# hassony2/handobjectconsist

Measured on AMD Instinct MI355X. Metric: trainmeshwarp iters/sec (render+warp, B=64, 256x256), higher is better.
Workload: dtype f32; 1 GPU; trainmeshwarp.py consist step, per-GPU B=64, 256x256, hand 778v/1552f + object 1002v/2000f (7104 faces after fill-back), ResNet-18 fp32 (MIOpen convolutions, channels-last, + fused HIP BatchNorm/ReLU/residual/max-pool kernels), Adam; global_batch=64, image_size=256, parallelism=dp1

## Files before the change

handobjectconsist_amd/csrc/frozen_bn.hip:

```cpp
#include "mr_common.hpp"

namespace mr {

__device__ __forceinline__ float relu_nan(float z) { return z > 0.0f ? z : (z != z ? z : 0.0f); }


struct BnParams {
    const void* x;
    const void* residual;
    const float* weight;
    const float* bias;
    const float* mean;
    const float* var;
    float eps;
    int relu;
    int N, C, HW, split;
    void* y;
    const void* grad_y;
    const void* grad_y2;
    void* grad_x;
    void* grad_residual;
    float* partial;
};

typedef unsigned short bf16_t;
__device__ __forceinline__ float to_f32(float v) { return v; }
__device__ __forceinline__ float to_f32(bf16_t v) { return __uint_as_float((unsigned)v << 16); }
template <typename T> __device__ __forceinline__ T from_f32(float v);
template <> __device__ __forceinline__ float from_f32<float>(float v) { return v; }
template <> __device__ __forceinline__ bf16_t from_f32<bf16_t>(float v) {
    unsigned u = __float_as_uint(v);
    if ((u & 0x7fffffffu) > 0x7f800000u) return (bf16_t)0x7fc0;
    u += 0x7fffu + ((u >> 16) & 1u);
    return (bf16_t)(u >> 16);
}
template <typename T> struct Vec4;
template <> struct Vec4<float> { typedef float4 type; };
template <> struct Vec4<bf16_t> { typedef ushort4 type; };

template <typename T>
__device__ __forceinline__ void load4(const void* base, int64_t o, float* v) {
    const typename Vec4<T>::type t = *reinterpret_cast<const typename Vec4<T>::type*>(static_cast<const T*>(base) + o);
    v[0] = to_f32(t.x); v[1] = to_f32(t.y); v[2] = to_f32(t.z); v[3] = to_f32(t.w);
}
template <typename T>
__device__ __forceinline__ void store4(void* base, int64_t o, const float* v) {
    typename Vec4<T>::type t;
    t.x = from_f32<T>(v[0]); t.y = from_f32<T>(v[1]); t.z = from_f32<T>(v[2]); t.w = from_f32<T>(v[3]);
    *reinterpret_cast<typename Vec4<T>::type*>(static_cast<T*>(base) + o) = t;
}

__device__ __forceinline__ void channel_consts(const BnParams& p, int c, float& mean, float& a, float& b, float& invstd) {
    mean = p.mean[c];
    invstd = 1.0f / sqrtf(p.var[c] + p.eps);
    a = p.weight[c] * invstd;
    b = p.bias[c];
}

template <typename T, bool VEC, bool BACKWARD>
__global__ __launch_bounds__(256) void bn_act_kernel(BnParams p) {
    const int c = blockIdx.x / p.split, k = blockIdx.x % p.split;
    const int n0 = (int)((int64_t)k * p.N / p.split), n1 = (int)((int64_t)(k + 1) * p.N / p.split);
    float mean, a, b, invstd;
    channel_consts(p, c, mean, a, b, invstd);
    constexpr int W = VEC ? 4 : 1;
    const int per_plane = p.HW / W;
    const unsigned total = (unsigned)(n1 - n0) * (unsigned)per_plane;
    const bool relu = p.relu != 0;
    float sum_g = 0.0f, sum_gx = 0.0f;
    for (unsigned e = threadIdx.x; e < total; e += 256) {
        const unsigned q = e / (unsigned)per_plane;
        const int n = n0 + (int)q, j = (int)(e - q * (unsigned)per_plane);
        const int64_t o = ((int64_t)n * p.C + c) * p.HW + (int64_t)j * W;
        float xv[W], rv[W], gv[W];
        if (VEC) {
            load4<T>(p.x, o, xv);
            if (p.residual) load4<T>(p.residual, o, rv);
            if (BACKWARD) {
                load4<T>(p.grad_y, o, gv);
                if (p.grad_y2) {
                    float g2[4];
                    load4<T>(p.grad_y2, o, g2);
#pragma unroll
                    for (int i = 0; i < 4; i++) gv[i] += g2[i];
                }
            }
        } else {
            xv[0] = to_f32(static_cast<const T*>(p.x)[o]);
            if (p.residual) rv[0] = to_f32(static_cast<const T*>(p.residual)[o]);
            if (BACKWARD) {
                gv[0] = to_f32(static_cast<const T*>(p.grad_y)[o]);
                if (p.grad_y2) gv[0] += to_f32(static_cast<const T*>(p.grad_y2)[o]);
            }
        }
        float out[W], gres[W];
#pragma unroll
        for (int i = 0; i < W; i++) {
            const float d = xv[i] - mean;
            float z = d * a + b;
            if (p.residual) z = z + rv[i];
            if (!BACKWARD) {
                out[i] = relu ? relu_nan(z) : z;
            } else {
                const float g = (relu && !(z > 0.0f)) ? 0.0f : gv[i];
                gres[i] = g;
                out[i] = g * a;
                sum_g += g;
                sum_gx += g * d;
            }
        }
        void* dst = BACKWARD ? p.grad_x : p.y;
        if (VEC) {
            store4<T>(dst, o, out);
            if (BACKWARD && p.grad_residual) store4<T>(p.grad_residual, o, gres);
        } else {
            static_cast<T*>(dst)[o] = from_f32<T>(out[0]);
            if (BACKWARD && p.grad_residual) static_cast<T*>(p.grad_residual)[o] = from_f32<T>(gres[0]);
        }
    }
    if (BACKWARD && p.partial) {
        __shared__ float red[2][4];
#pragma unroll
        for (int off = 32; off >= 1; off >>= 1) {
            sum_g += __shfl_down(sum_g, off);
            sum_gx += __shfl_down(sum_gx, off);
        }
        const int wave = threadIdx.x >> 6;
        if ((threadIdx.x & 63) == 0) { red[0][wave] = sum_g; red[1][wave] = sum_gx; }
        __syncthreads();
        if (threadIdx.x == 0) {
            p.partial[(int64_t)c * p.split + k] = (red[0][0] + red[0][1]) + (red[0][2] + red[0][3]);
            p.partial[(int64_t)(p.C + c) * p.split + k] = (red[1][0] + red[1][1]) + (red[1][2] + red[1][3]);
        }
    }
}

__global__ __launch_bounds__(256) void bn_finish_kernel(const float* __restrict__ partial, const float* __restrict__ var,
                                                        float eps, float* grad_weight, float* grad_bias, int C, int split) {
    __shared__ float red[2][4];
    const int c = blockIdx.x;
    float s0 = 0.0f, s1 = 0.0f;
    for (int k = threadIdx.x; k < split; k += 256) {
        s0 += partial[(int64_t)c * split + k];
        s1 += partial[(int64_t)(C + c) * split + k];
    }
#pragma unroll
    for (int off = 32; off >= 1; off >>= 1) {
        s0 += __shfl_down(s0, off);
        s1 += __shfl_down(s1, off);
    }
    if ((threadIdx.x & 63) == 0) { red[0][threadIdx.x >> 6] = s0; red[1][threadIdx.x >> 6] = s1; }
    __syncthreads();
    if (threadIdx.x == 0) {
        if (grad_bias) grad_bias[c] = (red[0][0] + red[0][1]) + (red[0][2] + red[0][3]);
        if (grad_weight) grad_weight[c] = ((red[1][0] + red[1][1]) + (red[1][2] + red[1][3])) * (1.0f / sqrtf(var[c] + eps));
    }
}

constexpr int BN_NHWC_BLOCKS = 2048;

template <typename T, bool BACKWARD>
__global__ __launch_bounds__(256) void bn_act_nhwc_kernel(BnParams p) {
    __shared__ float red[256][9];
    const int groups = p.C >> 2;
    const int cg = threadIdx.x % groups, prow = threadIdx.x / groups, rows = 256 / groups;
    const int c0 = 4 * cg;
    float mean[4], a[4], b[4];
#pragma unroll
    for (int i = 0; i < 4; i++) {
        float invstd;
        channel_consts(p, c0 + i, mean[i], a[i], b[i], invstd);
    }
    const int64_t pixels = (int64_t)p.N * p.HW;
    const bool relu = p.relu != 0;
    float sg[4] = {0.0f, 0.0f, 0.0f, 0.0f}, sgx[4] = {0.0f, 0.0f, 0.0f, 0.0f};
    for (int64_t px = (int64_t)blockIdx.x * rows + prow; px < pixels; px += (int64_t)gridDim.x * rows) {
        const int64_t o = px * p.C + c0;
        float xv[4], rv[4], gv[4], out[4], gres[4];
        load4<T>(p.x, o, xv);
        if (p.residual) load4<T>(p.residual, o, rv);
        if (BACKWARD) {
            load4<T>(p.grad_y, o, gv);
            if (p.grad_y2) {
                float g2[4];
                load4<T>(p.grad_y2, o, g2);
#pragma unroll
                for (int i = 0; i < 4; i++) gv[i] += g2[i];
            }
        }
#pragma unroll
        for (int i = 0; i < 4; i++) {
            const float d = xv[i] - mean[i];
            float z = d * a[i] + b[i];
            if (p.residual) z = z + rv[i];
            if (!BACKWARD) {
                out[i] = relu ? relu_nan(z) : z;
            } else {
                const float g = (relu && !(z > 0.0f)) ? 0.0f : gv[i];
                gres[i] = g;
                out[i] = g * a[i];
                sg[i] += g;
                sgx[i] += g * d;
            }
        }
        store4<T>(BACKWARD ? p.grad_x : p.y, o, out);
        if (BACKWARD && p.grad_residual) store4<T>(p.grad_residual, o, gres);
    }
    if (BACKWARD && p.partial) {
#pragma unroll
        for (int i = 0; i < 4; i++) { red[threadIdx.x][i] = sg[i]; red[threadIdx.x][4 + i] = sgx[i]; }
        __syncthreads();
        if (threadIdx.x < groups) {
            float t[8] = {0, 0, 0, 0, 0, 0, 0, 0};
            for (int r = 0; r < rows; r++)
#pragma unroll
                for (int i = 0; i < 8; i++) t[i] += red[r * groups + threadIdx.x][i];
#pragma unroll
            for (int i = 0; i < 4; i++) {
                p.partial[(int64_t)(c0 + i) * gridDim.x + blockIdx.x] = t[i];
                p.partial[(int64_t)(p.C + c0 + i) * gridDim.x + blockIdx.x] = t[4 + i];
            }
        }
    }
}

static inline bool bn_nhwc_ok(int C) { return C >= 4 && C <= 1024 && (1024 % C) == 0; }

static inline int bn_nhwc_blocks(int64_t pixels, int C) {
    const int rows = 256 / (C / 4);
    const int64_t need = (pixels + rows - 1) / rows;
    return (int)(need < BN_NHWC_BLOCKS ? (need < 1 ? 1 : need) : BN_NHWC_BLOCKS);
}

static inline int bn_split(int N, int C) {
    int s = (4096 + C - 1) / C;
    if (s < 1) s = 1;
    if (s > N) s = N;
    return s;
}

static inline bool bn_aligned(const void* p, int bytes) { return (reinterpret_cast<uintptr_t>(p) & (uintptr_t)(bytes - 1)) == 0; }

template <bool BACKWARD>
static void bn_launch(const BnParams& p, int act_dtype, bool vec, hipStream_t s) {
    const dim3 grid((unsigned)(p.C * p.split));
    if (act_dtype == 0) {
        if (vec) hipLaunchKernelGGL((bn_act_kernel<float, true, BACKWARD>), grid, dim3(256), 0, s, p);
        else hipLaunchKernelGGL((bn_act_kernel<float, false, BACKWARD>), grid, dim3(256), 0, s, p);
    } else {
        if (vec) hipLaunchKernelGGL((bn_act_kernel<bf16_t, true, BACKWARD>), grid, dim3(256), 0, s, p);
        else hipLaunchKernelGGL((bn_act_kernel<bf16_t, false, BACKWARD>), grid, dim3(256), 0, s, p);
    }
}

}

extern "C" int mr_bn_act_forward(const void* x, const void* residual, const float* weight, const float* bias,
                                 const float* running_mean, const float* running_var, float eps, int relu, int act_dtype,
                                 int channels_last, void* y, int batch_size, int channels, int plane,
                                 mr_stream_t stream) {
    using namespace mr;
    if (batch_size < 0 || channels < 0 || plane < 0 || (act_dtype != 0 && act_dtype != 1)) return MR_ERR_BADARG;
    if (channels_last && channels > 0 && !bn_nhwc_ok(channels)) return MR_ERR_BADARG;
    if (batch_size == 0 || channels == 0 || plane == 0) return MR_OK;
    if (!x || !weight || !bias || !running_mean || !running_var || !y) return MR_ERR_BADARG;
    BnParams p{};
    p.x = x; p.residual = residual; p.weight = weight; p.bias = bias; p.mean = running_mean; p.var = running_var;
    p.eps = eps; p.relu = relu; p.N = batch_size; p.C = channels; p.HW = plane; p.split = bn_split(batch_size, channels);
    p.y = y;
    if ((int64_t)channels * p.split > 0x7fffffff || ((int64_t)batch_size / p.split + 1) * plane > 0x7fffffff) return MR_ERR_BADARG;
    const int vb = act_dtype == 0 ? 16 : 8;
    if (channels_last) {
        if (!bn_aligned(x, vb) || !bn_aligned(y, vb) || !bn_aligned(residual, vb)) return MR_ERR_BADARG;
        const dim3 grid((unsigned)bn_nhwc_blocks((int64_t)batch_size * plane, channels));
        if (act_dtype == 0) hipLaunchKernelGGL((bn_act_nhwc_kernel<float, false>), grid, dim3(256), 0, (hipStream_t)stream, p);
        else hipLaunchKernelGGL((bn_act_nhwc_kernel<bf16_t, false>), grid, dim3(256), 0, (hipStream_t)stream, p);
        MR_CHECK_LAUNCH();
        return MR_OK;
    }
    const bool vec = plane % 4 == 0 && bn_aligned(x, vb) && bn_aligned(y, vb) && bn_aligned(residual, vb);
    bn_launch<false>(p, act_dtype, vec, (hipStream_t)stream);
    MR_CHECK_LAUNCH();
    return MR_OK;
}

extern "C" int64_t mr_bn_act_backward_workspace_bytes(int batch_size, int channels) {
    if (batch_size < 0 || channels < 0) return -1;
    const int64_t split = mr::bn_split(batch_size > 0 ? batch_size : 1, channels > 0 ? channels : 1);
    return (int64_t)2 * channels * (split > mr::BN_NHWC_BLOCKS ? split : mr::BN_NHWC_BLOCKS) * 4 + 16;
}

extern "C" int mr_bn_act_backward(const void* grad_y, const void* grad_y2, const void* x, const void* residual,
                                  const float* weight,
                                  const float* bias, const float* running_mean, const float* running_var, float eps,
                                  int relu, int act_dtype, int channels_last, void* grad_x, void* grad_residual,
                                  float* grad_weight, float* grad_bias, void* workspace, int64_t workspace_bytes,
                                  int batch_size, int channels, int plane, mr_stream_t stream) {
    using namespace mr;
    if (batch_size < 0 || channels < 0 || plane < 0 || (act_dtype != 0 && act_dtype != 1)) return MR_ERR_BADARG;
    if (channels_last && channels > 0 && !bn_nhwc_ok(channels)) return MR_ERR_BADARG;
    if (channels == 0) return MR_OK;
    if (!weight || !bias || !running_mean || !running_var) return MR_ERR_BADARG;
    const bool want_params = grad_weight || grad_bias;
    if (batch_size == 0 || plane == 0) {
        hipError_t e = hipSuccess;
        if (grad_weight) e = hipMemsetAsync(grad_weight, 0, (size_t)channels * 4, (hipStream_t)stream);
        if (e == hipSuccess && grad_bias) e = hipMemsetAsync(grad_bias, 0, (size_t)channels * 4, (hipStream_t)stream);
        return e == hipSuccess ? MR_OK : (int)e;
    }
    if (!grad_y || !x || !grad_x) return MR_ERR_BADARG;
    if (grad_residual && !residual) return MR_ERR_BADARG;
    if (want_params && (!workspace || workspace_bytes < mr_bn_act_backward_workspace_bytes(batch_size, channels)))
        return MR_ERR_BADARG;
    BnParams p{};
    p.x = x; p.residual = residual; p.weight = weight; p.bias = bias; p.mean = running_mean; p.var = running_var;
    p.eps = eps; p.relu = relu; p.N = batch_size; p.C = channels; p.HW = plane; p.split = bn_split(batch_size, channels);
    p.grad_y = grad_y; p.grad_y2 = grad_y2; p.grad_x = grad_x; p.grad_residual = grad_residual;
    p.partial = want_params ? static_cast<float*>(workspace) : nullptr;
    if ((int64_t)channels * p.split > 0x7fffffff || ((int64_t)batch_size / p.split + 1) * plane > 0x7fffffff) return MR_ERR_BADARG;
    const int vb = act_dtype == 0 ? 16 : 8;
    int slots = p.split;
    if (channels_last) {
        if (!bn_aligned(x, vb) || !bn_aligned(grad_y, vb) || !bn_aligned(grad_y2, vb) || !bn_aligned(grad_x, vb) ||
            !bn_aligned(residual, vb) ||
            !bn_aligned(grad_residual, vb))
            return MR_ERR_BADARG;
        slots = bn_nhwc_blocks((int64_t)batch_size * plane, channels);
        const dim3 grid((unsigned)slots);
        if (act_dtype == 0) hipLaunchKernelGGL((bn_act_nhwc_kernel<float, true>), grid, dim3(256), 0, (hipStream_t)stream, p);
        else hipLaunchKernelGGL((bn_act_nhwc_kernel<bf16_t, true>), grid, dim3(256), 0, (hipStream_t)stream, p);
    } else {
        const bool vec = plane % 4 == 0 && bn_aligned(x, vb) && bn_aligned(grad_y, vb) && bn_aligned(grad_y2, vb) &&
                         bn_aligned(grad_x, vb) &&
                         bn_aligned(residual, vb) && bn_aligned(grad_residual, vb);
        bn_launch<true>(p, act_dtype, vec, (hipStream_t)stream);
    }
    MR_CHECK_LAUNCH();
    if (want_params) {
        hipLaunchKernelGGL(bn_finish_kernel, dim3((unsigned)channels), dim3(256), 0, (hipStream_t)stream, p.partial,
                           running_var, eps, grad_weight, grad_bias, channels, slots);
        MR_CHECK_LAUNCH();
    }
    return MR_OK;
}
```

handobjectconsist_amd/csrc/stem_pool.hip:

```cpp
#include "mr_common.hpp"

namespace mr {

__device__ __forceinline__ float sp_relu_nan(float z) { return z > 0.0f ? z : (z != z ? z : 0.0f); }


struct StemParams {
    const void* x;
    const float* weight;
    const float* bias;
    const float* mean;
    const float* var;
    float eps;
    int N, C, H, W, OH, OW;
    int tiles_x, tiles_y;
    void* y;
    const void* grad_y;
    const void* grad_y2;
    void* grad_x;
    float* partial;
    unsigned char* argmax;
};

constexpr int SP_TX = 32, SP_TY = 16;
constexpr int SP_IH = 2 * SP_TY + 3, SP_IW = 2 * SP_TX + 8, SP_C0 = 4;
constexpr int SP_LDW = SP_IW + 1;

typedef unsigned short bf16_t;
__device__ __forceinline__ float sp_f32(float v) { return v; }
__device__ __forceinline__ float sp_f32(bf16_t v) { return __uint_as_float((unsigned)v << 16); }
template <typename T> __device__ __forceinline__ T sp_from(float v);
template <> __device__ __forceinline__ float sp_from<float>(float v) { return v; }
template <> __device__ __forceinline__ bf16_t sp_from<bf16_t>(float v) {
    unsigned u = __float_as_uint(v);
    if ((u & 0x7fffffffu) > 0x7f800000u) return (bf16_t)0x7fc0;
    u += 0x7fffu + ((u >> 16) & 1u);
    return (bf16_t)(u >> 16);
}
template <typename T> struct SpVec4;
template <> struct SpVec4<float> { typedef float4 type; };
template <> struct SpVec4<bf16_t> { typedef ushort4 type; };

__device__ __forceinline__ void stem_consts(const StemParams& p, int c, float& mean, float& a, float& b) {
    mean = p.mean[c];
    a = p.weight[c] * (1.0f / sqrtf(p.var[c] + p.eps));
    b = p.bias[c];
}

template <typename T, bool KEEP_D>
__device__ __forceinline__ void load_tile(const StemParams& p, const T* xp, int oy0, int ox0, float mean, float a,
                                          float b, float (*zt)[SP_LDW], float (*dt)[SP_LDW]) {
    const int iy0 = 2 * oy0 - 1, ix0 = 2 * ox0 - SP_C0;
    const float ninf = -__builtin_inff();
    if ((p.W & 3) == 0 && (reinterpret_cast<uintptr_t>(xp) & (4 * sizeof(T) - 1)) == 0) {
        for (int e = threadIdx.x; e < SP_IH * (SP_IW / 4); e += 256) {
            const int r = e / (SP_IW / 4), q = e - r * (SP_IW / 4);
            const int iy = iy0 + r, ix = ix0 + 4 * q;
            float v[4] = {0.0f, 0.0f, 0.0f, 0.0f};
            const bool in = iy >= 0 && iy < p.H && ix >= 0 && ix < p.W;
            if (in) {
                const typename SpVec4<T>::type t = *reinterpret_cast<const typename SpVec4<T>::type*>(xp + (int64_t)iy * p.W + ix);
                v[0] = sp_f32(t.x); v[1] = sp_f32(t.y); v[2] = sp_f32(t.z); v[3] = sp_f32(t.w);
            }
#pragma unroll
            for (int i = 0; i < 4; i++) {
                const float d = v[i] - mean;
                zt[r][4 * q + i] = in ? d * a + b : ninf;
                if (KEEP_D) dt[r][4 * q + i] = in ? d : 0.0f;
            }
        }
        return;
    }
    for (int e = threadIdx.x; e < SP_IH * SP_IW; e += 256) {
        const int r = e / SP_IW, c = e - r * SP_IW;
        const int iy = iy0 + r, ix = ix0 + c;
        float z = ninf, d = 0.0f;
        if (iy >= 0 && iy < p.H && ix >= 0 && ix < p.W) {
            d = sp_f32(xp[(int64_t)iy * p.W + ix]) - mean;
            z = d * a + b;
        }
        zt[r][c] = z;
        if (KEEP_D) dt[r][c] = d;
    }
}

template <typename T>
__global__ __launch_bounds__(256) void stem_pool_forward_kernel(StemParams p) {
    __shared__ float zt[SP_IH][SP_LDW];
    const int tiles = p.tiles_x * p.tiles_y;
    const int plane = blockIdx.x / tiles, t = blockIdx.x % tiles;
    const int c = plane % p.C;
    const int oy0 = (t / p.tiles_x) * SP_TY, ox0 = (t % p.tiles_x) * SP_TX;
    float mean, a, b;
    stem_consts(p, c, mean, a, b);
    load_tile<T, false>(p, static_cast<const T*>(p.x) + (int64_t)plane * p.H * p.W, oy0, ox0, mean, a, b, zt, nullptr);
    __syncthreads();
    for (int e = threadIdx.x; e < SP_TY * SP_TX; e += 256) {
        const int wy = e / SP_TX, wx = e % SP_TX;
        const int oy = oy0 + wy, ox = ox0 + wx;
        if (oy >= p.OH || ox >= p.OW) continue;
        float m = 0.0f;
#pragma unroll
        for (int kh = 0; kh < 3; kh++)
#pragma unroll
            for (int kw = 0; kw < 3; kw++) {
                const float z = zt[2 * wy + kh][2 * wx + kw + SP_C0 - 1];
                m = (z > m || z != z) ? z : m;
            }
        static_cast<T*>(p.y)[((int64_t)plane * p.OH + oy) * p.OW + ox] = sp_from<T>(m);
    }
}

template <typename T>
__global__ __launch_bounds__(256) void stem_pool_backward_kernel(StemParams p) {
    __shared__ float zt[SP_IH][SP_LDW];
    __shared__ float dt[SP_IH][SP_LDW];
    __shared__ float gw[SP_TY + 1][SP_TX + 1];
    __shared__ unsigned char am[SP_TY + 1][SP_TX + 1];
    __shared__ float red[2][4];
    const int tiles = p.tiles_x * p.tiles_y;
    const int plane = blockIdx.x / tiles, t = blockIdx.x % tiles;
    const int c = plane % p.C;
    const int oy0 = (t / p.tiles_x) * SP_TY, ox0 = (t % p.tiles_x) * SP_TX;
    float mean, a, b;
    stem_consts(p, c, mean, a, b);
    const T* xp = static_cast<const T*>(p.x) + (int64_t)plane * p.H * p.W;
    load_tile<T, true>(p, xp, oy0, ox0, mean, a, b, zt, dt);
    __syncthreads();
    for (int e = threadIdx.x; e < (SP_TY + 1) * (SP_TX + 1); e += 256) {
        const int wy = e / (SP_TX + 1), wx = e - wy * (SP_TX + 1);
        const int oy = oy0 + wy, ox = ox0 + wx;
        float g = 0.0f;
        int best = 0;
        if (oy < p.OH && ox < p.OW) {
            g = sp_f32(static_cast<const T*>(p.grad_y)[((int64_t)plane * p.OH + oy) * p.OW + ox]);
            if (p.grad_y2) g += sp_f32(static_cast<const T*>(p.grad_y2)[((int64_t)plane * p.OH + oy) * p.OW + ox]);
            float mv = -__builtin_inff();
#pragma unroll
            for (int k = 0; k < 9; k++) {
                const float z = zt[2 * wy + k / 3][2 * wx + k % 3 + SP_C0 - 1];
                const float v = sp_relu_nan(z);
                if (z != -__builtin_inff() && (v > mv || v != v)) { mv = v; best = k; }
            }
        }
        gw[wy][wx] = g;
        am[wy][wx] = (unsigned char)best;
    }
    __syncthreads();
    float sum_g = 0.0f, sum_gx = 0.0f;
    T* gx = static_cast<T*>(p.grad_x) + (int64_t)plane * p.H * p.W;
    const bool vec = (p.W & 3) == 0 && (reinterpret_cast<uintptr_t>(gx) & (4 * sizeof(T) - 1)) == 0;
    for (int e = threadIdx.x; e < 2 * SP_TY * (2 * SP_TX / 4); e += 256) {
        const int ry = e / (2 * SP_TX / 4), rx0 = 4 * (e - ry * (2 * SP_TX / 4));
        const int iy = 2 * oy0 + ry, ix0 = 2 * ox0 + rx0;
        if (iy >= p.H || ix0 >= p.W) continue;
        const int ly = ry + 1;
        float out[4];
#pragma unroll
        for (int i = 0; i < 4; i++) {
            const int lx = rx0 + i + 1;
            float g = 0.0f;
#pragma unroll
            for (int dy = 0; dy < 2; dy++) {
                const int wy = (ly >> 1) - dy;
                const int kh = ly - 2 * wy;
                if (wy < 0 || kh > 2) continue;
#pragma unroll
                for (int dx = 0; dx < 2; dx++) {
                    const int wx = (lx >> 1) - dx;
                    const int kw = lx - 2 * wx;
                    if (wx < 0 || kw > 2) continue;
                    if (am[wy][wx] == kh * 3 + kw) g += gw[wy][wx];
                }
            }
            const float z = zt[ly][lx + SP_C0 - 1];
            const float gm = (z > 0.0f && ix0 + i < p.W) ? g : 0.0f;
            out[i] = gm * a;
            sum_g += gm;
            sum_gx += gm * dt[ly][lx + SP_C0 - 1];
        }
        T* dst = gx + (int64_t)iy * p.W + ix0;
        if (vec) {
            typename SpVec4<T>::type t;
            t.x = sp_from<T>(out[0]); t.y = sp_from<T>(out[1]); t.z = sp_from<T>(out[2]); t.w = sp_from<T>(out[3]);
            *reinterpret_cast<typename SpVec4<T>::type*>(dst) = t;
        } else {
#pragma unroll
            for (int i = 0; i < 4; i++)
                if (ix0 + i < p.W) dst[i] = sp_from<T>(out[i]);
        }
    }
    if (p.partial) {
#pragma unroll
        for (int off = 32; off >= 1; off >>= 1) {
            sum_g += __shfl_down(sum_g, off);
            sum_gx += __shfl_down(sum_gx, off);
        }
        const int wave = threadIdx.x >> 6;
        if ((threadIdx.x & 63) == 0) { red[0][wave] = sum_g; red[1][wave] = sum_gx; }
        __syncthreads();
        if (threadIdx.x == 0) {
            const int n = plane / p.C;
            const int64_t per_c = (int64_t)p.N * tiles;
            const int64_t slot = (int64_t)n * tiles + t;
            p.partial[(int64_t)c * per_c + slot] = (red[0][0] + red[0][1]) + (red[0][2] + red[0][3]);
            p.partial[((int64_t)p.C + c) * per_c + slot] = (red[1][0] + red[1][1]) + (red[1][2] + red[1][3]);
        }
    }
}

__global__ __launch_bounds__(256) void stem_finish_kernel(const float* __restrict__ partial, const float* __restrict__ var,
                                                          float eps, float* grad_weight, float* grad_bias, int C,
                                                          int64_t per_c) {
    __shared__ float red[2][4];
    const int c = blockIdx.x;
    float s0 = 0.0f, s1 = 0.0f;
    for (int64_t k = threadIdx.x; k < per_c; k += 256) {
        s0 += partial[(int64_t)c * per_c + k];
        s1 += partial[((int64_t)C + c) * per_c + k];
    }
#pragma unroll
    for (int off = 32; off >= 1; off >>= 1) {
        s0 += __shfl_down(s0, off);
        s1 += __shfl_down(s1, off);
    }
    if ((threadIdx.x & 63) == 0) { red[0][threadIdx.x >> 6] = s0; red[1][threadIdx.x >> 6] = s1; }
    __syncthreads();
    if (threadIdx.x == 0) {
        if (grad_bias) grad_bias[c] = (red[0][0] + red[0][1]) + (red[0][2] + red[0][3]);
        if (grad_weight) grad_weight[c] = ((red[1][0] + red[1][1]) + (red[1][2] + red[1][3])) * (1.0f / sqrtf(var[c] + eps));
    }
}

constexpr int SP_NHWC_BLOCKS = 4096;

template <typename T>
__device__ __forceinline__ void sp_load4(const T* base, int64_t o, float* v) {
    const typename SpVec4<T>::type t = *reinterpret_cast<const typename SpVec4<T>::type*>(base + o);
    v[0] = sp_f32(t.x); v[1] = sp_f32(t.y); v[2] = sp_f32(t.z); v[3] = sp_f32(t.w);
}
template <typename T>
__device__ __forceinline__ void sp_store4(T* base, int64_t o, const float* v) {
    typename SpVec4<T>::type t;
    t.x = sp_from<T>(v[0]); t.y = sp_from<T>(v[1]); t.z = sp_from<T>(v[2]); t.w = sp_from<T>(v[3]);
    *reinterpret_cast<typename SpVec4<T>::type*>(base + o) = t;
}

template <typename T>
__global__ __launch_bounds__(256) void stem_pool_nhwc_forward_kernel(StemParams p) {
    const int groups = p.C >> 2, cg = threadIdx.x % groups, prow = threadIdx.x / groups, rows = 256 / groups;
    const int c0 = 4 * cg;
    float mean[4], a[4], b[4];
#pragma unroll
    for (int i = 0; i < 4; i++) stem_consts(p, c0 + i, mean[i], a[i], b[i]);
    const T* x = static_cast<const T*>(p.x);
    const int64_t total = (int64_t)p.N * p.OH * p.OW;
    for (int64_t op = (int64_t)blockIdx.x * rows + prow; op < total; op += (int64_t)gridDim.x * rows) {
        const int ox = (int)(op % p.OW), oy = (int)((op / p.OW) % p.OH), n = (int)(op / ((int64_t)p.OW * p.OH));
        float best[4];
        unsigned bi[4] = {0, 0, 0, 0};
#pragma unroll
        for (int i = 0; i < 4; i++) best[i] = -__builtin_inff();
#pragma unroll
        for (int k = 0; k < 9; k++) {
            const int iy = 2 * oy - 1 + k / 3, ix = 2 * ox - 1 + k % 3;
            if (iy < 0 || iy >= p.H || ix < 0 || ix >= p.W) continue;
            float xv[4];
            sp_load4<T>(x, (((int64_t)n * p.H + iy) * p.W + ix) * p.C + c0, xv);
#pragma unroll
            for (int i = 0; i < 4; i++) {
                const float v = sp_relu_nan((xv[i] - mean[i]) * a[i] + b[i]);
                if (v > best[i] || v != v) { best[i] = v; bi[i] = (unsigned)k; }
            }
        }
        const int64_t o = op * p.C + c0;
        sp_store4<T>(static_cast<T*>(p.y), o, best);
        *reinterpret_cast<uchar4*>(p.argmax + o) = make_uchar4((unsigned char)bi[0], (unsigned char)bi[1],
                                                               (unsigned char)bi[2], (unsigned char)bi[3]);
    }
}

template <typename T>
__global__ __launch_bounds__(256) void stem_pool_nhwc_backward_kernel(StemParams p) {
    __shared__ float red[256][9];
    const int groups = p.C >> 2, cg = threadIdx.x % groups, prow = threadIdx.x / groups, rows = 256 / groups;
    const int c0 = 4 * cg;
    float mean[4], a[4], b[4];
#pragma unroll
    for (int i = 0; i < 4; i++) stem_consts(p, c0 + i, mean[i], a[i], b[i]);
    const T* x = static_cast<const T*>(p.x);
    const T* gy = static_cast<const T*>(p.grad_y);
    const T* gy2 = static_cast<const T*>(p.grad_y2);
    const int64_t total = (int64_t)p.N * p.H * p.W;
    float sg[4] = {0.0f, 0.0f, 0.0f, 0.0f}, sgx[4] = {0.0f, 0.0f, 0.0f, 0.0f};
    for (int64_t ip = (int64_t)blockIdx.x * rows + prow; ip < total; ip += (int64_t)gridDim.x * rows) {
        const int ix = (int)(ip % p.W), iy = (int)((ip / p.W) % p.H), n = (int)(ip / ((int64_t)p.W * p.H));
        float xv[4], g[4] = {0.0f, 0.0f, 0.0f, 0.0f}, out[4];
        sp_load4<T>(x, ip * p.C + c0, xv);
        const int ly = iy + 1, lx = ix + 1;
#pragma unroll
        for (int dy = 0; dy < 2; dy++) {
            const int wy = (ly >> 1) - dy, kh = ly - 2 * wy;
            if (wy < 0 || wy >= p.OH || kh > 2) continue;
#pragma unroll
            for (int dx = 0; dx < 2; dx++) {
                const int wx = (lx >> 1) - dx, kw = lx - 2 * wx;
                if (wx < 0 || wx >= p.OW || kw > 2) continue;
                const int64_t o = (((int64_t)n * p.OH + wy) * p.OW + wx) * p.C + c0;
                const uchar4 id = *reinterpret_cast<const uchar4*>(p.argmax + o);
                float gv[4];
                sp_load4<T>(gy, o, gv);
                if (gy2) {
                    float g2[4];
                    sp_load4<T>(gy2, o, g2);
#pragma unroll
                    for (int i = 0; i < 4; i++) gv[i] += g2[i];
                }
                const unsigned code = (unsigned)(kh * 3 + kw);
                g[0] += id.x == code ? gv[0] : 0.0f;
                g[1] += id.y == code ? gv[1] : 0.0f;
                g[2] += id.z == code ? gv[2] : 0.0f;
                g[3] += id.w == code ? gv[3] : 0.0f;
            }
        }
#pragma unroll
        for (int i = 0; i < 4; i++) {
            const float d = xv[i] - mean[i];
            const float gm = (d * a[i] + b[i] > 0.0f) ? g[i] : 0.0f;
            out[i] = gm * a[i];
            sg[i] += gm;
            sgx[i] += gm * d;
        }
        sp_store4<T>(static_cast<T*>(p.grad_x), ip * p.C + c0, out);
    }
    if (p.partial) {
#pragma unroll
        for (int i = 0; i < 4; i++) { red[threadIdx.x][i] = sg[i]; red[threadIdx.x][4 + i] = sgx[i]; }
        __syncthreads();
        if (threadIdx.x < groups) {
            float t[8] = {0, 0, 0, 0, 0, 0, 0, 0};
            for (int r = 0; r < rows; r++)
#pragma unroll
                for (int i = 0; i < 8; i++) t[i] += red[r * groups + threadIdx.x][i];
#pragma unroll
            for (int i = 0; i < 4; i++) {
                p.partial[(int64_t)(c0 + i) * gridDim.x + blockIdx.x] = t[i];
                p.partial[(int64_t)(p.C + c0 + i) * gridDim.x + blockIdx.x] = t[4 + i];
            }
        }
    }
}

static inline bool sp_nhwc_ok(int C) { return C >= 4 && C <= 1024 && (1024 % C) == 0; }
static inline int sp_nhwc_blocks(int64_t pixels, int C) {
    const int rows = 256 / (C / 4);
    const int64_t need = (pixels + rows - 1) / rows;
    return (int)(need < SP_NHWC_BLOCKS ? (need < 1 ? 1 : need) : SP_NHWC_BLOCKS);
}

static int stem_fill(StemParams& p, const void* x, const float* weight, const float* bias, const float* mean,
                     const float* var, float eps, int N, int C, int H, int W) {
    if (N < 0 || C < 0 || H < 0 || W < 0) return MR_ERR_BADARG;
    p.x = x; p.weight = weight; p.bias = bias; p.mean = mean; p.var = var; p.eps = eps;
    p.N = N; p.C = C; p.H = H; p.W = W;
    p.OH = H > 0 ? (H - 1) / 2 + 1 : 0;
    p.OW = W > 0 ? (W - 1) / 2 + 1 : 0;
    p.tiles_x = (p.OW + SP_TX - 1) / SP_TX;
    p.tiles_y = (p.OH + SP_TY - 1) / SP_TY;
    if ((int64_t)N * C * p.tiles_x * p.tiles_y > 0x7fffffff) return MR_ERR_BADARG;
    return MR_OK;
}

}

extern "C" int mr_stem_pool_forward(const void* x, const float* weight, const float* bias, const float* running_mean,
                                    const float* running_var, float eps, int act_dtype, int channels_last, void* y,
                                    unsigned char* argmax, int batch_size, int channels, int height, int width,
                                    mr_stream_t stream) {
    using namespace mr;
    if (act_dtype != 0 && act_dtype != 1) return MR_ERR_BADARG;
    if (channels_last && channels > 0 && !sp_nhwc_ok(channels)) return MR_ERR_BADARG;
    StemParams p{};
    const int rc = stem_fill(p, x, weight, bias, running_mean, running_var, eps, batch_size, channels, height, width);
    if (rc != MR_OK) return rc;
    if (batch_size == 0 || channels == 0 || height == 0 || width == 0) return MR_OK;
    if (!x || !weight || !bias || !running_mean || !running_var || !y) return MR_ERR_BADARG;
    p.y = y;
    if (channels_last) {
        const uintptr_t am = (uintptr_t)(act_dtype == 0 ? 15 : 7);
        if (!argmax || (reinterpret_cast<uintptr_t>(x) & am) || (reinterpret_cast<uintptr_t>(y) & am) ||
            (reinterpret_cast<uintptr_t>(argmax) & 3))
            return MR_ERR_BADARG;
        p.argmax = argmax;
        const dim3 g((unsigned)sp_nhwc_blocks((int64_t)batch_size * p.OH * p.OW, channels));
        if (act_dtype == 0) hipLaunchKernelGGL(stem_pool_nhwc_forward_kernel<float>, g, dim3(256), 0, (hipStream_t)stream, p);
        else hipLaunchKernelGGL(stem_pool_nhwc_forward_kernel<bf16_t>, g, dim3(256), 0, (hipStream_t)stream, p);
        MR_CHECK_LAUNCH();
        return MR_OK;
    }
    const dim3 grid((unsigned)((int64_t)batch_size * channels * p.tiles_x * p.tiles_y));
    if (act_dtype == 0) hipLaunchKernelGGL(stem_pool_forward_kernel<float>, grid, dim3(256), 0, (hipStream_t)stream, p);
    else hipLaunchKernelGGL(stem_pool_forward_kernel<bf16_t>, grid, dim3(256), 0, (hipStream_t)stream, p);
    MR_CHECK_LAUNCH();
    return MR_OK;
}

extern "C" int64_t mr_stem_pool_backward_workspace_bytes(int batch_size, int channels, int height, int width) {
    using namespace mr;
    StemParams p{};
    if (stem_fill(p, nullptr, nullptr, nullptr, nullptr, nullptr, 0.0f, batch_size, channels, height, width) != MR_OK) return -1;
    const int64_t nchw = (int64_t)batch_size * p.tiles_x * p.tiles_y;
    return (int64_t)2 * channels * (nchw > SP_NHWC_BLOCKS ? nchw : SP_NHWC_BLOCKS) * 4 + 16;
}

extern "C" int mr_stem_pool_backward(const void* grad_y, const void* grad_y2, const void* x, const unsigned char* argmax,
                                     const float* weight, const float* bias, const float* running_mean, const float* running_var, float eps,
                                     int act_dtype, int channels_last, void* grad_x, float* grad_weight,
                                     float* grad_bias, void* workspace, int64_t workspace_bytes, int batch_size,
                                     int channels, int height, int width, mr_stream_t stream) {
    using namespace mr;
    if (act_dtype != 0 && act_dtype != 1) return MR_ERR_BADARG;
    if (channels_last && channels > 0 && !sp_nhwc_ok(channels)) return MR_ERR_BADARG;
    StemParams p{};
    const int rc = stem_fill(p, x, weight, bias, running_mean, running_var, eps, batch_size, channels, height, width);
    if (rc != MR_OK) return rc;
    if (channels == 0) return MR_OK;
    const bool want_params = grad_weight || grad_bias;
    if (batch_size == 0 || height == 0 || width == 0) {
        hipError_t e = hipSuccess;
        if (grad_weight) e = hipMemsetAsync(grad_weight, 0, (size_t)channels * 4, (hipStream_t)stream);
        if (e == hipSuccess && grad_bias) e = hipMemsetAsync(grad_bias, 0, (size_t)channels * 4, (hipStream_t)stream);
        return e == hipSuccess ? MR_OK : (int)e;
    }
    if (!grad_y || !x || !weight || !bias || !running_mean || !running_var || !grad_x) return MR_ERR_BADARG;
    if (want_params &&
        (!workspace || workspace_bytes < mr_stem_pool_backward_workspace_bytes(batch_size, channels, height, width)))
        return MR_ERR_BADARG;
    p.grad_y = grad_y; p.grad_y2 = grad_y2; p.grad_x = grad_x;
    p.partial = want_params ? static_cast<float*>(workspace) : nullptr;
    const int tiles = p.tiles_x * p.tiles_y;
    int64_t slots = (int64_t)batch_size * tiles;
    if (channels_last) {
        const uintptr_t am = (uintptr_t)(act_dtype == 0 ? 15 : 7);
        if (!argmax || (reinterpret_cast<uintptr_t>(x) & am) || (reinterpret_cast<uintptr_t>(grad_y) & am) ||
            (reinterpret_cast<uintptr_t>(grad_y2) & am) ||
            (reinterpret_cast<uintptr_t>(grad_x) & am) || (reinterpret_cast<uintptr_t>(argmax) & 3))
            return MR_ERR_BADARG;
        p.argmax = const_cast<unsigned char*>(argmax);
        slots = sp_nhwc_blocks((int64_t)batch_size * height * width, channels);
        const dim3 g((unsigned)slots);
        if (act_dtype == 0) hipLaunchKernelGGL(stem_pool_nhwc_backward_kernel<float>, g, dim3(256), 0, (hipStream_t)stream, p);
        else hipLaunchKernelGGL(stem_pool_nhwc_backward_kernel<bf16_t>, g, dim3(256), 0, (hipStream_t)stream, p);
    } else {
        const dim3 grid((unsigned)((int64_t)batch_size * channels * tiles));
        if (act_dtype == 0) hipLaunchKernelGGL(stem_pool_backward_kernel<float>, grid, dim3(256), 0, (hipStream_t)stream, p);
        else hipLaunchKernelGGL(stem_pool_backward_kernel<bf16_t>, grid, dim3(256), 0, (hipStream_t)stream, p);
    }
    MR_CHECK_LAUNCH();
    if (want_params) {
        hipLaunchKernelGGL(stem_finish_kernel, dim3((unsigned)channels), dim3(256), 0, (hipStream_t)stream, p.partial,
                           running_var, eps, grad_weight, grad_bias, channels, slots);
        MR_CHECK_LAUNCH();
    }
    return MR_OK;
}
```

Before: 37.43 iters/s (one optimiser step = 1 data batch + 1 consist batch of B per GPU; roofline.stock_trunk_it_s = the same step with the trunk's BatchNorm/ReLU/max-pool on the stock nn modules).

## Restructure NHWC BN and stem-pool backward with shared window reuse and row-major partials

The NHWC BatchNorm backward now processes two pixels per thread per trip, and its grid is sized from a trip count clamped to a minimum block count. Per-block channel sums are reduced with wave shuffles and LDS and written as contiguous per-block rows, which a new vectorised finish kernel consumes. The stem max-pool backward is rewritten to walk 2x2 input quads along a row segment and reuse the loaded pooling windows (argmax and grad) between neighbours, instead of reloading up to four windows per input pixel. The aim is less redundant global traffic and cheaper reductions in these backward kernels, at the cost of more register pressure, fewer blocks, and a new 16-byte workspace alignment requirement.

Result: faster. 37.84 iters/s (one optimiser step = 1 data batch + 1 consist batch of B per GPU; roofline.stock_trunk_it_s = the same step with the trunk's BatchNorm/ReLU/max-pool on the stock nn modules), median of 6 (+1.1%).

```diff
diff --git a/handobjectconsist_amd/csrc/channel_sums.hpp b/handobjectconsist_amd/csrc/channel_sums.hpp
--- /dev/null
+++ b/handobjectconsist_amd/csrc/channel_sums.hpp
@@ -0,0 +1,68 @@
+#pragma once
+#include "mr_common.hpp"
+
+namespace mr {
+
+constexpr int CS_LDS_FLOATS = 2048;
+
+__device__ __forceinline__ void block_channel_sums(float* s, int groups, int C, float* lds, float* __restrict__ row) {
+#pragma unroll
+    for (int off = 32; off >= 1; off >>= 1) {
+        if (off >= groups) {
+#pragma unroll
+            for (int i = 0; i < 8; i++) s[i] += __shfl_xor(s[i], off);
+        }
+    }
+    const int lane = threadIdx.x & 63, wave = threadIdx.x >> 6;
+    const int per_wave = groups < 64 ? groups : 64;
+    const int lds_rows = groups <= 64 ? 4 : 256 / groups;
+    if (lane < per_wave) {
+        const int r = groups <= 64 ? wave : (int)threadIdx.x / groups;
+        const int g = groups <= 64 ? lane % groups : (int)threadIdx.x % groups;
+        float* dst = lds + ((size_t)r * groups + g) * 8;
+        *reinterpret_cast<float4*>(dst) = make_float4(s[0], s[1], s[2], s[3]);
+        *reinterpret_cast<float4*>(dst + 4) = make_float4(s[4], s[5], s[6], s[7]);
+    }
+    __syncthreads();
+    for (int t = threadIdx.x; t < 2 * groups; t += 256) {
+        const int g = t % groups, half = t / groups;
+        float4 acc = *reinterpret_cast<const float4*>(lds + (size_t)g * 8 + 4 * half);
+        for (int r = 1; r < lds_rows; r++) {
+            const float4 v = *reinterpret_cast<const float4*>(lds + ((size_t)r * groups + g) * 8 + 4 * half);
+            acc.x += v.x; acc.y += v.y; acc.z += v.z; acc.w += v.w;
+        }
+        *reinterpret_cast<float4*>(row + (size_t)half * C + 4 * g) = acc;
+    }
+}
+
+__device__ __forceinline__ void finish_channel_sums(const float* __restrict__ partial, const float* __restrict__ var,
+                                                    float eps, float* grad_weight, float* grad_bias, int C, int64_t slots) {
+    __shared__ float red[4][4];
+    const int j = 4 * blockIdx.x;
+    const int cw = j + (int)(threadIdx.x & 3) - C;
+    const float scale = cw >= 0 ? 1.0f / sqrtf(var[cw] + eps) : 1.0f;
+    float4 s = make_float4(0.0f, 0.0f, 0.0f, 0.0f);
+    for (int64_t k = threadIdx.x; k < slots; k += 256) {
+        const float4 v = *reinterpret_cast<const float4*>(partial + k * (2 * C) + j);
+        s.x += v.x; s.y += v.y; s.z += v.z; s.w += v.w;
+    }
+#pragma unroll
+    for (int off = 32; off >= 1; off >>= 1) {
+        s.x += __shfl_xor(s.x, off); s.y += __shfl_xor(s.y, off);
+        s.z += __shfl_xor(s.z, off); s.w += __shfl_xor(s.w, off);
+    }
+    const int wave = threadIdx.x >> 6;
+    if ((threadIdx.x & 63) == 0) { red[wave][0] = s.x; red[wave][1] = s.y; red[wave][2] = s.z; red[wave][3] = s.w; }
+    __syncthreads();
+    if (threadIdx.x < 4) {
+        const int i = threadIdx.x, c = j + i;
+        const float t = (red[0][i] + red[1][i]) + (red[2][i] + red[3][i]);
+        if (c < C) {
+            if (grad_bias) grad_bias[c] = t;
+        } else if (grad_weight) {
+            grad_weight[c - C] = t * scale;
+        }
+    }
+}
+
+}
diff --git a/handobjectconsist_amd/csrc/frozen_bn.hip b/handobjectconsist_amd/csrc/frozen_bn.hip
--- a/handobjectconsist_amd/csrc/frozen_bn.hip
+++ b/handobjectconsist_amd/csrc/frozen_bn.hip
@@ -1,4 +1,5 @@
 #include "mr_common.hpp"
+#include "channel_sums.hpp"
 
 namespace mr {
 
@@ -158,10 +159,13 @@
 }
 
 constexpr int BN_NHWC_BLOCKS = 2048;
+constexpr int BN_NHWC_MIN_BLOCKS = 1024;
+constexpr int BN_NHWC_BWD_PX = 2, BN_NHWC_BWD_TRIPS = 4;
 
 template <typename T, bool BACKWARD>
 __global__ __launch_bounds__(256) void bn_act_nhwc_kernel(BnParams p) {
-    __shared__ float red[256][9];
+    constexpr int PX = BACKWARD ? BN_NHWC_BWD_PX : 1;
+    __shared__ __attribute__((aligned(16))) float lds[CS_LDS_FLOATS];
     const int groups = p.C >> 2;
     const int cg = threadIdx.x % groups, prow = threadIdx.x / groups, rows = 256 / groups;
     const int c0 = 4 * cg;
@@ -172,64 +176,73 @@
         channel_consts(p, c0 + i, mean[i], a[i], b[i], invstd);
     }
     const int64_t pixels = (int64_t)p.N * p.HW;
+    const int64_t stride = (int64_t)gridDim.x * rows;
     const bool relu = p.relu != 0;
-    float sg[4] = {0.0f, 0.0f, 0.0f, 0.0f}, sgx[4] = {0.0f, 0.0f, 0.0f, 0.0f};
-    for (int64_t px = (int64_t)blockIdx.x * rows + prow; px < pixels; px += (int64_t)gridDim.x * rows) {
-        const int64_t o = px * p.C + c0;
-        float xv[4], rv[4], gv[4], out[4], gres[4];
-        load4<T>(p.x, o, xv);
-        if (p.residual) load4<T>(p.residual, o, rv);
-        if (BACKWARD) {
-            load4<T>(p.grad_y, o, gv);
-            if (p.grad_y2) {
-                float g2[4];
-                load4<T>(p.grad_y2, o, g2);
-#pragma unroll
-                for (int i = 0; i < 4; i++) gv[i] += g2[i];
-            }
-        }
-#pragma unroll
-        for (int i = 0; i < 4; i++) {
-            const float d = xv[i] - mean[i];
-            float z = d * a[i] + b[i];
-            if (p.residual) z = z + rv[i];
-            if (!BACKWARD) {
-                out[i] = relu ? relu_nan(z) : z;
-            } else {
-                const float g = (relu && !(z > 0.0f)) ? 0.0f : gv[i];
-                gres[i] = g;
-                out[i] = g * a[i];
-                sg[i] += g;
-                sgx[i] += g * d;
-            }
-        }
-        store4<T>(BACKWARD ? p.grad_x : p.y, o, out);
-        if (BACKWARD && p.grad_residual) store4<T>(p.grad_residual, o, gres);
-    }
-    if (BACKWARD && p.partial) {
-#pragma unroll
-        for (int i = 0; i < 4; i++) { red[threadIdx.x][i] = sg[i]; red[threadIdx.x][4 + i] = sgx[i]; }
-        __syncthreads();
-        if (threadIdx.x < groups) {
-            float t[8] = {0, 0, 0, 0, 0, 0, 0, 0};
-            for (int r = 0; r < rows; r++)
-#pragma unroll
-                for (int i = 0; i < 8; i++) t[i] += red[r * groups + threadIdx.x][i];
+    float s[8] = {0.0f, 0.0f, 0.0f, 0.0f, 0.0f, 0.0f, 0.0f, 0.0f};
+    for (int64_t px = (int64_t)blockIdx.x * rows + prow; px < pixels; px += PX * stride) {
+        float xv[PX][4], rv[PX][4], gv[PX][4];
+        bool live[PX];
+#pragma unroll
+        for (int u = 0; u < PX; u++) {
+            live[u] = px + u * stride < pixels;
+            if (!live[u]) continue;
+            const int64_t o = (px + u * stride) * p.C + c0;
+            load4<T>(p.x, o, xv[u]);
+            if (p.residual) load4<T>(p.residual, o, rv[u]);
+            if (BACKWARD) {
+                load4<T>(p.grad_y, o, gv[u]);
+                if (p.grad_y2) {
+                    float g2[4];
+                    load4<T>(p.grad_y2, o, g2);
+#pragma unroll
+                    for (int i = 0; i < 4; i++) gv[u][i] += g2[i];
+                }
+            }
+        }
+#pragma unroll
+        for (int u = 0; u < PX; u++) {
+            if (!live[u]) continue;
+            const int64_t o = (px + u * stride) * p.C + c0;
+            float out[4], gres[4];
 #pragma unroll
             for (int i = 0; i < 4; i++) {
-                p.partial[(int64_t)(c0 + i) * gridDim.x + blockIdx.x] = t[i];
-                p.partial[(int64_t)(p.C + c0 + i) * gridDim.x + blockIdx.x] = t[4 + i];
-            }
-        }
-    }
+                const float d = xv[u][i] - mean[i];
+                float z = d * a[i] + b[i];
+                if (p.residual) z = z + rv[u][i];
+                if (!BACKWARD) {
+                    out[i] = relu ? relu_nan(z) : z;
+                } else {
+                    const float g = (relu && !(z > 0.0f)) ? 0.0f : gv[u][i];
+                    gres[i] = g;
+                    out[i] = g * a[i];
+                    s[i] += g;
+                    s[4 + i] += g * d;
+                }
+            }
+            store4<T>(BACKWARD ? p.grad_x : p.y, o, out);
+            if (BACKWARD && p.grad_residual) store4<T>(p.grad_residual, o, gres);
+        }
+    }
+    if (BACKWARD && p.partial) block_channel_sums(s, groups, p.C, lds, p.partial + (size_t)blockIdx.x * 2 * p.C);
+}
+
+__global__ __launch_bounds__(256) void bn_finish_nhwc_kernel(const float* __restrict__ partial,
+                                                                           const float* __restrict__ var, float eps,
+                                                                           float* grad_weight, float* grad_bias, int C,
+                                                                           int slots) {
+    finish_channel_sums(partial, var, eps, grad_weight, grad_bias, C, slots);
 }
 
 static inline bool bn_nhwc_ok(int C) { return C >= 4 && C <= 1024 && (1024 % C) == 0; }
 
-static inline int bn_nhwc_blocks(int64_t pixels, int C) {
-    const int rows = 256 / (C / 4);
-    const int64_t need = (pixels + rows - 1) / rows;
-    return (int)(need < BN_NHWC_BLOCKS ? (need < 1 ? 1 : need) : BN_NHWC_BLOCKS);
+static inline int bn_nhwc_blocks(int64_t pixels, int C, int px, int trips) {
+    const int64_t per_trip = (int64_t)(256 / (C / 4)) * px;
+    const int64_t need = (pixels + per_trip - 1) / per_trip;
+    int64_t g = need / trips;
+    if (g < BN_NHWC_MIN_BLOCKS) g = BN_NHWC_MIN_BLOCKS;
+    if (g > BN_NHWC_BLOCKS) g = BN_NHWC_BLOCKS;
+    if (g > need) g = need;
+    return (int)(g < 1 ? 1 : g);
 }
 
 static inline int bn_split(int N, int C) {
@@ -272,7 +285,7 @@
     const int vb = act_dtype == 0 ? 16 : 8;
     if (channels_last) {
         if (!bn_aligned(x, vb) || !bn_aligned(y, vb) || !bn_aligned(residual, vb)) return MR_ERR_BADARG;
-        const dim3 grid((unsigned)bn_nhwc_blocks((int64_t)batch_size * plane, channels));
+        const dim3 grid((unsigned)bn_nhwc_blocks((int64_t)batch_size * plane, channels, 1, 1));
         if (act_dtype == 0) hipLaunchKernelGGL((bn_act_nhwc_kernel<float, false>), grid, dim3(256), 0, (hipStream_t)stream, p);
         else hipLaunchKernelGGL((bn_act_nhwc_kernel<bf16_t, false>), grid, dim3(256), 0, (hipStream_t)stream, p);
         MR_CHECK_LAUNCH();
@@ -323,9 +336,9 @@
     if (channels_last) {
         if (!bn_aligned(x, vb) || !bn_aligned(grad_y, vb) || !bn_aligned(grad_y2, vb) || !bn_aligned(grad_x, vb) ||
             !bn_aligned(residual, vb) ||
-            !bn_aligned(grad_residual, vb))
+            !bn_aligned(grad_residual, vb) || !bn_aligned(workspace, 16))
             return MR_ERR_BADARG;
-        slots = bn_nhwc_blocks((int64_t)batch_size * plane, channels);
+        slots = bn_nhwc_blocks((int64_t)batch_size * plane, channels, BN_NHWC_BWD_PX, BN_NHWC_BWD_TRIPS);
         const dim3 grid((unsigned)slots);
         if (act_dtype == 0) hipLaunchKernelGGL((bn_act_nhwc_kernel<float, true>), grid, dim3(256), 0, (hipStream_t)stream, p);
         else hipLaunchKernelGGL((bn_act_nhwc_kernel<bf16_t, true>), grid, dim3(256), 0, (hipStream_t)stream, p);
@@ -336,7 +349,11 @@
         bn_launch<true>(p, act_dtype, vec, (hipStream_t)stream);
     }
     MR_CHECK_LAUNCH();
-    if (want_params) {
+    if (want_params && channels_last) {
+        hipLaunchKernelGGL(bn_finish_nhwc_kernel, dim3((unsigned)(channels / 2)), dim3(256), 0, (hipStream_t)stream, p.partial, running_var, eps, grad_weight,
+                           grad_bias, channels, slots);
+        MR_CHECK_LAUNCH();
+    } else if (want_params) {
         hipLaunchKernelGGL(bn_finish_kernel, dim3((unsigned)channels), dim3(256), 0, (hipStream_t)stream, p.partial,
                            running_var, eps, grad_weight, grad_bias, channels, slots);
         MR_CHECK_LAUNCH();
diff --git a/handobjectconsist_amd/csrc/stem_pool.hip b/handobjectconsist_amd/csrc/stem_pool.hip
--- a/handobjectconsist_amd/csrc/stem_pool.hip
+++ b/handobjectconsist_amd/csrc/stem_pool.hip
@@ -1,4 +1,5 @@
 #include "mr_common.hpp"
+#include "channel_sums.hpp"
 
 namespace mr {
 
@@ -232,7 +233,9 @@
     }
 }
 
-constexpr int SP_NHWC_BLOCKS = 4096;
+constexpr int SP_NHWC_FWD_BLOCKS = 4096;
+constexpr int SP_NHWC_BLOCKS = 2048, SP_NHWC_MIN_BLOCKS = 1024, SP_NHWC_TRIPS = 3;
+constexpr int SP_BWD_RUN = 4;
 
 template <typename T>
 __device__ __forceinline__ void sp_load4(const T* base, int64_t o, float* v) {
@@ -280,82 +283,134 @@
     }
 }
 
+struct SpWindow {
+    float g[4];
+    unsigned code;
+};
+__device__ __forceinline__ float sp_take(const SpWindow& w, int i, unsigned code) {
+    return ((w.code >> (8 * i)) & 255u) == code ? w.g[i] : 0.0f;
+}
+
 template <typename T>
 __global__ __launch_bounds__(256) void stem_pool_nhwc_backward_kernel(StemParams p) {
-    __shared__ float red[256][9];
+    __shared__ __attribute__((aligned(16))) float lds[CS_LDS_FLOATS];
     const int groups = p.C >> 2, cg = threadIdx.x % groups, prow = threadIdx.x / groups, rows = 256 / groups;
     const int c0 = 4 * cg;
     float mean[4], a[4], b[4];
 #pragma unroll
     for (int i = 0; i < 4; i++) stem_consts(p, c0 + i, mean[i], a[i], b[i]);
-    const T* x = static_cast<const T*>(p.x);
-    const T* gy = static_cast<const T*>(p.grad_y);
-    const T* gy2 = static_cast<const T*>(p.grad_y2);
-    const int64_t total = (int64_t)p.N * p.H * p.W;
-    float sg[4] = {0.0f, 0.0f, 0.0f, 0.0f}, sgx[4] = {0.0f, 0.0f, 0.0f, 0.0f};
-    for (int64_t ip = (int64_t)blockIdx.x * rows + prow; ip < total; ip += (int64_t)gridDim.x * rows) {
-        const int ix = (int)(ip % p.W), iy = (int)((ip / p.W) % p.H), n = (int)(ip / ((int64_t)p.W * p.H));
-        float xv[4], g[4] = {0.0f, 0.0f, 0.0f, 0.0f}, out[4];
-        sp_load4<T>(x, ip * p.C + c0, xv);
-        const int ly = iy + 1, lx = ix + 1;
-#pragma unroll
-        for (int dy = 0; dy < 2; dy++) {
-            const int wy = (ly >> 1) - dy, kh = ly - 2 * wy;
-            if (wy < 0 || wy >= p.OH || kh > 2) continue;
-#pragma unroll
-            for (int dx = 0; dx < 2; dx++) {
-                const int wx = (lx >> 1) - dx, kw = lx - 2 * wx;
-                if (wx < 0 || wx >= p.OW || kw > 2) continue;
-                const int64_t o = (((int64_t)n * p.OH + wy) * p.OW + wx) * p.C + c0;
-                const uchar4 id = *reinterpret_cast<const uchar4*>(p.argmax + o);
-                float gv[4];
-                sp_load4<T>(gy, o, gv);
-                if (gy2) {
-                    float g2[4];
-                    sp_load4<T>(gy2, o, g2);
-#pragma unroll
-                    for (int i = 0; i < 4; i++) gv[i] += g2[i];
+    const T* __restrict__ x = static_cast<const T*>(p.x);
+    const T* __restrict__ gy = static_cast<const T*>(p.grad_y);
+    const T* __restrict__ gy2 = static_cast<const T*>(p.grad_y2);
+    const unsigned char* __restrict__ am = p.argmax;
+    T* __restrict__ gx = static_cast<T*>(p.grad_x);
+    const int QH = (p.H + 1) >> 1, QW = (p.W + 1) >> 1, segs = (QW + SP_BWD_RUN - 1) / SP_BWD_RUN;
+    const int64_t items = (int64_t)p.N * QH * segs;
+    float s[8] = {0.0f, 0.0f, 0.0f, 0.0f, 0.0f, 0.0f, 0.0f, 0.0f};
+    for (int64_t it = (int64_t)blockIdx.x * rows + prow; it < items; it += (int64_t)gridDim.x * rows) {
+        const int seg = (int)(it % segs), q = (int)((it / segs) % QH), n = (int)(it / ((int64_t)segs * QH));
+        const int p0 = seg * SP_BWD_RUN, p1 = min(p0 + SP_BWD_RUN, QW);
+        const bool low = q + 1 < p.OH;
+        const bool row1 = 2 * q + 1 < p.H;
+        auto load_win = [&](SpWindow& w, int wy, int wx, bool ok) {
+            if (!ok) {
+                w.g[0] = w.g[1] = w.g[2] = w.g[3] = 0.0f;
+                w.code = 0xffffffffu;
+                return;
+            }
+            const int64_t o = (((int64_t)n * p.OH + wy) * p.OW + wx) * p.C + c0;
+            w.code = *reinterpret_cast<const unsigned*>(am + o);
+            sp_load4<T>(gy, o, w.g);
+            if (gy2) {
+                float g2[4];
+                sp_load4<T>(gy2, o, g2);
+#pragma unroll
+                for (int i = 0; i < 4; i++) w.g[i] += g2[i];
+            }
+        };
+        auto finish = [&](int iy, int ix, const float* xv, const float* g) {
+            float out[4];
+#pragma unroll
+            for (int i = 0; i < 4; i++) {
+                const float d = xv[i] - mean[i];
+                const float gm = (d * a[i] + b[i] > 0.0f) ? g[i] : 0.0f;
+                out[i] = gm * a[i];
+                s[i] += gm;
+                s[4 + i] += gm * d;
+            }
+            sp_store4<T>(gx, (((int64_t)n * p.H + iy) * p.W + ix) * p.C + c0, out);
+        };
+        SpWindow a0, b0;
+        load_win(a0, q, p0, true);
+        load_win(b0, q + 1, p0, low);
+        for (int pq = p0; pq < p1; pq++) {
+            const bool right = pq + 1 < p.OW;
+            const bool col1 = 2 * pq + 1 < p.W;
+            SpWindow a1, b1;
+            load_win(a1, q, pq + 1, right);
+            load_win(b1, q + 1, pq + 1, right && low);
+            const int64_t xo = (((int64_t)n * p.H + 2 * q) * p.W + 2 * pq) * p.C + c0;
+            float x00[4], x01[4], x10[4], x11[4];
+            sp_load4<T>(x, xo, x00);
+            if (col1) sp_load4<T>(x, xo + p.C, x01);
+            if (row1) sp_load4<T>(x, xo + (int64_t)p.W * p.C, x10);
+            if (row1 && col1) sp_load4<T>(x, xo + (int64_t)p.W * p.C + p.C, x11);
+            float g[4];
+#pragma unroll
+            for (int i = 0; i < 4; i++) { g[i] = 0.0f; g[i] += sp_take(a0, i, 4); }
+            finish(2 * q, 2 * pq, x00, g);
+            if (col1) {
+#pragma unroll
+                for (int i = 0; i < 4; i++) { g[i] = 0.0f; g[i] += sp_take(a1, i, 3); g[i] += sp_take(a0, i, 5); }
+                finish(2 * q, 2 * pq + 1, x01, g);
+            }
+            if (row1) {
+#pragma unroll
+                for (int i = 0; i < 4; i++) { g[i] = 0.0f; g[i] += sp_take(b0, i, 1); g[i] += sp_take(a0, i, 7); }
+                finish(2 * q + 1, 2 * pq, x10, g);
+            }
+            if (row1 && col1) {
+#pragma unroll
+                for (int i = 0; i < 4; i++) {
+                    g[i] = 0.0f;
+                    g[i] += sp_take(b1, i, 0);
+                    g[i] += sp_take(b0, i, 2);
+                    g[i] += sp_take(a1, i, 6);
+                    g[i] += sp_take(a0, i, 8);
                 }
-                const unsigned code = (unsigned)(kh * 3 + kw);
-                g[0] += id.x == code ? gv[0] : 0.0f;
-                g[1] += id.y == code ? gv[1] : 0.0f;
-                g[2] += id.z == code ? gv[2] : 0.0f;
-                g[3] += id.w == code ? gv[3] : 0.0f;
-            }
-        }
-#pragma unroll
-        for (int i = 0; i < 4; i++) {
-            const float d = xv[i] - mean[i];
-            const float gm = (d * a[i] + b[i] > 0.0f) ? g[i] : 0.0f;
-            out[i] = gm * a[i];
-            sg[i] += gm;
-            sgx[i] += gm * d;
-        }
-        sp_store4<T>(static_cast<T*>(p.grad_x), ip * p.C + c0, out);
-    }
-    if (p.partial) {
-#pragma unroll
-        for (int i = 0; i < 4; i++) { red[threadIdx.x][i] = sg[i]; red[threadIdx.x][4 + i] = sgx[i]; }
-        __syncthreads();
-        if (threadIdx.x < groups) {
-            float t[8] = {0, 0, 0, 0, 0, 0, 0, 0};
-            for (int r = 0; r < rows; r++)
-#pragma unroll
-                for (int i = 0; i < 8; i++) t[i] += red[r * groups + threadIdx.x][i];
-#pragma unroll
-            for (int i = 0; i < 4; i++) {
-                p.partial[(int64_t)(c0 + i) * gridDim.x + blockIdx.x] = t[i];
-                p.partial[(int64_t)(p.C + c0 + i) * gridDim.x + blockIdx.x] = t[4 + i];
-            }
-        }
-    }
+                finish(2 * q + 1, 2 * pq + 1, x11, g);
+            }
+            a0 = a1;
+            b0 = b1;
+        }
+    }
+    if (p.partial) block_channel_sums(s, groups, p.C, lds, p.partial + (size_t)blockIdx.x * 2 * p.C);
+}
+
+__global__ __launch_bounds__(256) void stem_finish_nhwc_kernel(const float* __restrict__ partial,
+                                                                             const float* __restrict__ var, float eps,
+                                                                             float* grad_weight, float* grad_bias, int C,
+                                                                             int slots) {
+    finish_channel_sums(partial, var, eps, grad_weight, grad_bias, C, slots);
 }
 
 static inline bool sp_nhwc_ok(int C) { return C >= 4 && C <= 1024 && (1024 % C) == 0; }
-static inline int sp_nhwc_blocks(int64_t pixels, int C) {
+static inline int sp_nhwc_blocks(int64_t items, int C) {
+    const int rows = 256 / (C / 4);
+    const int64_t need = (items + rows - 1) / rows;
+    int64_t g = need / SP_NHWC_TRIPS;
+    if (g < SP_NHWC_MIN_BLOCKS) g = SP_NHWC_MIN_BLOCKS;
+    if (g > SP_NHWC_BLOCKS) g = SP_NHWC_BLOCKS;
+    if (g > need) g = need;
+    return (int)(g < 1 ? 1 : g);
+}
+static inline int sp_nhwc_fwd_blocks(int64_t pixels, int C) {
     const int rows = 256 / (C / 4);
     const int64_t need = (pixels + rows - 1) / rows;
-    return (int)(need < SP_NHWC_BLOCKS ? (need < 1 ? 1 : need) : SP_NHWC_BLOCKS);
+    return (int)(need < SP_NHWC_FWD_BLOCKS ? (need < 1 ? 1 : need) : SP_NHWC_FWD_BLOCKS);
+}
+static inline int64_t sp_bwd_items(const StemParams& p) {
+    return (int64_t)p.N * p.OH * ((p.OW + SP_BWD_RUN - 1) / SP_BWD_RUN);
 }
 
 static int stem_fill(StemParams& p, const void* x, const float* weight, const float* bias, const float* mean,
@@ -392,7 +447,7 @@
             (reinterpret_cast<uintptr_t>(argmax) & 3))
             return MR_ERR_BADARG;
         p.argmax = argmax;
-        const dim3 g((unsigned)sp_nhwc_blocks((int64_t)batch_size * p.OH * p.OW, channels));
+        const dim3 g((unsigned)sp_nhwc_fwd_blocks((int64_t)batch_size * p.OH * p.OW, channels));
         if (act_dtype == 0) hipLaunchKernelGGL(stem_pool_nhwc_forward_kernel<float>, g, dim3(256), 0, (hipStream_t)stream, p);
         else hipLaunchKernelGGL(stem_pool_nhwc_forward_kernel<bf16_t>, g, dim3(256), 0, (hipStream_t)stream, p);
         MR_CHECK_LAUNCH();
@@ -444,10 +499,11 @@
         const uintptr_t am = (uintptr_t)(act_dtype == 0 ? 15 : 7);
         if (!argmax || (reinterpret_cast<uintptr_t>(x) & am) || (reinterpret_cast<uintptr_t>(grad_y) & am) ||
             (reinterpret_cast<uintptr_t>(grad_y2) & am) ||
-            (reinterpret_cast<uintptr_t>(grad_x) & am) || (reinterpret_cast<uintptr_t>(argmax) & 3))
+            (reinterpret_cast<uintptr_t>(grad_x) & am) || (reinterpret_cast<uintptr_t>(argmax) & 3) ||
+            (reinterpret_cast<uintptr_t>(workspace) & 15))
             return MR_ERR_BADARG;
         p.argmax = const_cast<unsigned char*>(argmax);
-        slots = sp_nhwc_blocks((int64_t)batch_size * height * width, channels);
+        slots = sp_nhwc_blocks(sp_bwd_items(p), channels);
         const dim3 g((unsigned)slots);
         if (act_dtype == 0) hipLaunchKernelGGL(stem_pool_nhwc_backward_kernel<float>, g, dim3(256), 0, (hipStream_t)stream, p);
         else hipLaunchKernelGGL(stem_pool_nhwc_backward_kernel<bf16_t>, g, dim3(256), 0, (hipStream_t)stream, p);
@@ -457,7 +513,11 @@
         else hipLaunchKernelGGL(stem_pool_backward_kernel<bf16_t>, grid, dim3(256), 0, (hipStream_t)stream, p);
     }
     MR_CHECK_LAUNCH();
-    if (want_params) {
+    if (want_params && channels_last) {
+        hipLaunchKernelGGL(stem_finish_nhwc_kernel, dim3((unsigned)(channels / 2)), dim3(256), 0, (hipStream_t)stream, p.partial, running_var, eps, grad_weight,
+                           grad_bias, channels, (int)slots);
+        MR_CHECK_LAUNCH();
+    } else if (want_params) {
         hipLaunchKernelGGL(stem_finish_kernel, dim3((unsigned)channels), dim3(256), 0, (hipStream_t)stream, p.partial,
                            running_var, eps, grad_weight, grad_bias, channels, slots);
         MR_CHECK_LAUNCH();
```
